# opas-lab/olearning-sim

Measured on AMD Instinct MI355X. Metric: virtual clients/sec (simulated FL rounds, FedAvg CNN), higher is better.
Workload: dtype bfloat16; 1 GPU; model=resnet18, preset=resnet-10k, clients_total=1250, clients_per_gpu=1250, local_steps=2, local_batch=16, num_classes=100, parallelism=dp1, global_batch=20000

## Files before the change

### olearning_sim_amd/models/resnet.py

```python

from __future__ import annotations

from typing import Optional

import torch

from .base import (ClientBatchedModel, Params, binit, kaiming,
                   blinear, bconv2d)

_STAGES = (64, 128, 256, 512)
_GN_GROUPS = 8


class ResNet18(ClientBatchedModel):
    name = "resnet18"
    num_classes = 100
    act_elems_per_sample = 1_600_000
    input_shape = (3, 32, 32)

    def __init__(self, num_classes: int = 100, in_ch: int = 3,
                 width_mult: float = 1.0):
        self.num_classes = num_classes
        self.in_ch = in_ch
        self.widths = [int(w * width_mult) for w in _STAGES]
# ... 27 lines not shown
                    conv(f"{pre}.down", out_c, ic, 1)
                    gn(f"{pre}.gndown", out_c)
            in_c = out_c
        p["fc.w"] = binit((w[3], self.num_classes), w[3], device, dtype, g)
        p["fc.b"] = binit((self.num_classes,), w[3], device, dtype, g)
        return p

    def _block(self, params: Params, x: torch.Tensor, C: int, pre: str,
               stride: int, has_down: bool) -> torch.Tensor:
        from ..ops.fused import groupnorm_act
        h = bconv2d(x, params[f"{pre}.c1.w"], C, stride=stride, padding=1)
        h = groupnorm_act(h, C, _GN_GROUPS, params[f"{pre}.gn1.g"],
                          params[f"{pre}.gn1.b"], relu=True)
        h = bconv2d(h, params[f"{pre}.c2.w"], C, stride=1, padding=1)
        if has_down:
            sc = bconv2d(x, params[f"{pre}.down.w"], C, stride=stride)
            sc = groupnorm_act(sc, C, _GN_GROUPS, params[f"{pre}.gndown.g"],
                               params[f"{pre}.gndown.b"])
        else:
            sc = x
        return groupnorm_act(h, C, _GN_GROUPS, params[f"{pre}.gn2.g"],
                             params[f"{pre}.gn2.b"], res=sc, relu=True)

    def _block_cbf(self, params: Params, x: torch.Tensor, C: int, pre: str,
                   stride: int, has_down: bool) -> torch.Tensor:
        from ..ops.conv import client_conv3x3, client_conv1x1
        from ..ops.fused import groupnorm_act
        h = client_conv3x3(x, params[f"{pre}.c1.w"], stride)
        h = groupnorm_act(h, C, _GN_GROUPS, params[f"{pre}.gn1.g"],
                          params[f"{pre}.gn1.b"], relu=True)
        h = client_conv3x3(h, params[f"{pre}.c2.w"], 1)
        if has_down:
            sc = client_conv1x1(x, params[f"{pre}.down.w"], stride)
            sc = groupnorm_act(sc, C, _GN_GROUPS, params[f"{pre}.gndown.g"],
                               params[f"{pre}.gndown.b"])
        else:
            sc = x
        return groupnorm_act(h, C, _GN_GROUPS, params[f"{pre}.gn2.g"],
                             params[f"{pre}.gn2.b"], res=sc, relu=True)

    def forward_cbf(self, params: Params, x: torch.Tensor) -> torch.Tensor:
        from ..ops.conv import client_conv3x3
        from ..ops.fused import groupnorm_act
        C, B = x.shape[0], x.shape[1]
        h = x.permute(0, 2, 1, 3, 4).contiguous()
        h = client_conv3x3(h, params["stem.w"], 1)
        h = groupnorm_act(h, C, _GN_GROUPS, params["stem.gn.g"],
                          params["stem.gn.b"], relu=True)
        for s in range(4):
            stride = 1 if s == 0 else 2
            h = self._block_cbf(params, h, C, f"s{s}.b0", stride, s > 0)
            h = self._block_cbf(params, h, C, f"s{s}.b1", 1, False)
        h = h.mean(dim=(3, 4)).permute(0, 2, 1)
        return blinear(h, params["fc.w"], params["fc.b"])

    def forward(self, params: Params, x: torch.Tensor) -> torch.Tensor:
        from ..ops.fused import groupnorm_act
        import os
        if x.is_cuda and x.dtype == torch.bfloat16 and \
                os.environ.get("OLSIM_CONV", "custom") == "custom":
            from ..ops.fused import hip_ops_available
            if hip_ops_available():
                return self.forward_cbf(params, x)
        C, B = x.shape[0], x.shape[1]
        h = x.permute(1, 0, 2, 3, 4).reshape(B, C * self.in_ch, 32, 32)
        h = bconv2d(h, params["stem.w"], C, stride=1, padding=1)
        h = groupnorm_act(h, C, _GN_GROUPS, params["stem.gn.g"],
                          params["stem.gn.b"], relu=True)
        for s in range(4):
            stride = 1 if s == 0 else 2
            has_down = s > 0
            h = self._block(params, h, C, f"s{s}.b0", stride, has_down)
            h = self._block(params, h, C, f"s{s}.b1", 1, False)
        h = h.mean(dim=(2, 3)).reshape(B, C, self.widths[3]).permute(1, 0, 2)
        return blinear(h, params["fc.w"], params["fc.b"])
# ... 1 lines not shown
```

### olearning_sim_amd/ops/conv.py

```python

from __future__ import annotations

import torch
import torch.nn.functional as F

from .fused import load_hip_ops


def _cpu_conv3x3(x: torch.Tensor, w: torch.Tensor, stride: int) -> torch.Tensor:
    C, IC, B, H, W = x.shape
    OC = w.shape[1]
    xg = x.permute(2, 0, 1, 3, 4).reshape(B, C * IC, H, W)
    wf = w.reshape(C * OC, IC, 3, 3)
    y = F.conv2d(xg, wf, stride=stride, padding=1, groups=C)
    OH, OW = y.shape[-2:]
    return y.reshape(B, C, OC, OH, OW).permute(1, 2, 0, 3, 4).contiguous()


class _Conv3x3Fn(torch.autograd.Function):
    @staticmethod
    def forward(ctx, x, w, stride):
        ops = load_hip_ops(required=True)
        y = ops.conv3x3_fwd(x, w, stride)
        ctx.save_for_backward(x, w)
# ... 27 lines not shown

    @staticmethod
    def forward(ctx, x, w, stride):
        ops = load_hip_ops(required=True)
        x_pad = _pad(x, 1)
        y = ops.conv3x3_fwd_p(x_pad, w, stride)
        ctx.save_for_backward(x_pad, w)
        ctx.stride = stride
        return y

    @staticmethod
    def backward(ctx, dy):
        x_pad, w = ctx.saved_tensors
        ops = load_hip_ops(required=True)
        dy = dy.contiguous()
        dx = dw = None
        H, W = x_pad.shape[3] - 2, x_pad.shape[4] - 2
        if ctx.needs_input_grad[0]:
            dy_pad = _pad(dy, 1)
            dx = ops.conv3x3_dgrad_p(dy_pad, w, H, W, ctx.stride)
        if ctx.needs_input_grad[1]:
            dw = ops.conv3x3_wgrad_p(x_pad, dy, ctx.stride)
        return dx, dw, None


def _v6_ok(ops, x: torch.Tensor, w: torch.Tensor, stride: int) -> bool:
    import os
    if os.environ.get("OLSIM_CONV_V", "") == "5":
        return False
    C, IC, B, H, W = x.shape
    return bool(ops.conv3x3_v6_ok(IC, w.shape[1], B, H, W, stride))


def client_conv3x3(x: torch.Tensor, w: torch.Tensor,
                   stride: int = 1) -> torch.Tensor:
    if x.is_cuda and x.dtype == torch.bfloat16:
        ops = load_hip_ops(required=True)
        if _v6_ok(ops, x, w, stride):
            return _Conv3x3PadFn.apply(x.contiguous(), w.contiguous(), stride)
        return _Conv3x3Fn.apply(x.contiguous(), w.contiguous(), stride)
    return _cpu_conv3x3(x, w, stride)



_NTAB_CACHE: dict = {}

# ... 94 lines not shown
    if x.is_cuda and x.dtype in (torch.bfloat16, torch.float32):
        return _Pool2x2Fn.apply(x.contiguous())
    shape = x.shape
    flat = x.reshape(-1, 1, shape[-2], shape[-1])
    out = F.max_pool2d(flat, 2)
    return out.reshape(*shape[:-2], shape[-2] // 2, shape[-1] // 2)


class _Subsample2Fn(torch.autograd.Function):

    @staticmethod
    def forward(ctx, x):
        ops = load_hip_ops(required=True)
        ctx.hw = x.shape[-2:]
        return ops.subsample2(x.contiguous())

    @staticmethod
    def backward(ctx, dy):
        ops = load_hip_ops(required=True)
        H, W = ctx.hw
        return ops.subsample2_bwd(dy.contiguous(), H, W)


def client_conv1x1(x: torch.Tensor, w: torch.Tensor,
                   stride: int = 1) -> torch.Tensor:
    C, IC, B, H, W = x.shape
    OC = w.shape[1]
    if stride != 1:
        if (stride == 2 and x.is_cuda and H % 2 == 0 and W % 4 == 0
                and x.dtype in (torch.bfloat16, torch.float32)):
            x = _Subsample2Fn.apply(x)
        else:
            x = x[:, :, :, ::stride, ::stride].contiguous()
        H, W = x.shape[-2:]
    y = torch.bmm(w.reshape(C, OC, IC), x.reshape(C, IC, B * H * W))
    return y.view(C, OC, B, H, W)
```

### olearning_sim_amd/ops/csrc/bindings.cpp

```cpp

#include <torch/extension.h>
#include <ATen/cuda/CUDAContext.h>
#include <hip/hip_runtime.h>

extern "C" void ols_fused_sgd_update_flat(
    void* buf, const void* grad, const void* master, const int64_t* offs,
    int nblocks, int64_t clients, int64_t total, float lr, float mu,
    int dtype, hipStream_t stream);

extern "C" void ols_weighted_delta_accum_flat(
    float* delta, const void* buf, const void* master, const float* weights,
    const int64_t* offs, int nblocks, int64_t clients, int64_t pglobal,
    float wsum, int dtype, hipStream_t stream);

extern "C" void ols_cross_entropy_fwd_bwd(
    const void* logits, const int64_t* labels, float* loss, void* dlogits,
    int64_t nrows, int64_t K, float inv_n, int dtype, hipStream_t stream);

extern "C" void ols_groupnorm_fwd(const void* x, const void* res, void* y,
                                  float* mean, float* rstd, const void* gamma,
                                  const void* beta, int B, int C, int ch,
                                  int G, int HW, float eps, bool relu,
                                  int layout, int dtype, hipStream_t stream);

// ... 63 lines not shown

extern "C" void ols_relu_mask(const void* dy, const void* y, void* out,
                              int64_t n, int dtype, hipStream_t stream);

extern "C" void ols_layernorm_fwd(const void* x, const void* gamma,
                                  const void* beta, void* y, float* mean,
                                  float* rstd, int64_t rows, int H,
                                  int64_t rows_per_client, float eps,
                                  int dtype, hipStream_t stream);
extern "C" void ols_layernorm_bwd(const void* x, const void* dy,
                                  const void* gamma, const float* mean,
                                  const float* rstd, void* dx, float* dgamma,
                                  float* dbeta, int64_t rows, int H,
                                  int64_t rows_per_client, int dtype,
                                  hipStream_t stream);

extern "C" void ols_groupnorm_bwd(const void* x, const void* y,
                                  const void* dy, void* dx, void* dres,
                                  const float* mean, const float* rstd,
                                  const void* gamma, float* dgamma,
                                  float* dbeta, int B, int C, int ch, int G,
                                  int HW, bool relu, int layout, int dtype,
                                  hipStream_t stream);

namespace {

int dtype_code(const at::Tensor& t) {
  switch (t.scalar_type()) {
    case at::kFloat: return 0;
    case at::kBFloat16: return 1;
    case at::kHalf: return 2;
    default:
      TORCH_CHECK(false, "olsim_hip: unsupported dtype ", t.scalar_type());
  }
}

void fused_sgd_update_flat(at::Tensor buf, at::Tensor grad,
                           at::Tensor global_flat, at::Tensor offsets,
                           int64_t clients, double lr, double mu) {
  TORCH_CHECK(buf.is_cuda() && buf.is_contiguous(), "buf must be GPU+contig");
  TORCH_CHECK(grad.sizes() == buf.sizes() && grad.scalar_type() == buf.scalar_type());
  const bool prox = mu != 0.0 && global_flat.numel() > 0;
  if (prox) {
    TORCH_CHECK(offsets.numel() >= 2 && offsets.scalar_type() == at::kLong);
    TORCH_CHECK(global_flat.scalar_type() == buf.scalar_type());
  }
// ... 348 lines not shown
  int64_t planes = x.numel() / ((int64_t)H * W);
  auto sizes = x.sizes().vec();
  sizes[sizes.size() - 2] = H / 2;
  sizes[sizes.size() - 1] = W / 2;
  auto y = at::empty(sizes, x.options());
  int dt = x.scalar_type() == at::kBFloat16 ? 1 : 0;
  ols_subsample2_fwd(x.data_ptr(), y.data_ptr(), planes, H / 2, W / 2, dt,
                     at::cuda::getCurrentCUDAStream().stream());
  return y;
}

at::Tensor subsample2_bwd(at::Tensor dy, int64_t H, int64_t W) {
  TORCH_CHECK(dy.is_cuda() && dy.is_contiguous() && dy.dim() >= 2);
  TORCH_CHECK(dy.size(-2) == H / 2 && dy.size(-1) == W / 2);
  int64_t planes = dy.numel() / ((int64_t)(H / 2) * (W / 2));
  auto sizes = dy.sizes().vec();
  sizes[sizes.size() - 2] = H;
  sizes[sizes.size() - 1] = W;
  auto dx = at::empty(sizes, dy.options());
  int dt = dy.scalar_type() == at::kBFloat16 ? 1 : 0;
  ols_subsample2_bwd(dy.data_ptr(), dx.data_ptr(), planes, (int)H, (int)W,
                     dt, at::cuda::getCurrentCUDAStream().stream());
  return dx;
}


at::Tensor replicate(at::Tensor src, int64_t clients) {
  TORCH_CHECK(src.is_cuda() && src.is_contiguous() && clients >= 1);
  TORCH_CHECK(src.numel() % 8 == 0);
  TORCH_CHECK(src.scalar_type() == at::kBFloat16 ||
              src.scalar_type() == at::kFloat);
  auto sizes = src.sizes().vec();
  sizes.insert(sizes.begin(), clients);
  auto dst = at::empty(sizes, src.options());
  int dt = src.scalar_type() == at::kBFloat16 ? 1 : 0;
  ols_replicate(src.data_ptr(), dst.data_ptr(), clients, src.numel(), dt,
                at::cuda::getCurrentCUDAStream().stream());
  return dst;
}

at::Tensor synth_batch(at::Tensor x, at::Tensor y, double s, double t) {
  TORCH_CHECK(x.is_cuda() && x.is_contiguous() && x.dim() == 2);
  TORCH_CHECK(x.scalar_type() == at::kFloat && x.size(1) % 8 == 0);
  TORCH_CHECK(y.is_cuda() && y.is_contiguous() &&
              y.scalar_type() == at::kLong);
  int64_t rows = y.numel(), batch = x.size(0), n = x.size(1);
// ... 64 lines not shown
  m.def("groupnorm_bwd(Tensor x, Tensor y, Tensor dy, Tensor mean, "
        "Tensor rstd, Tensor gamma, int clients, int groups, bool has_res, "
        "bool relu) -> (Tensor, Tensor, Tensor, Tensor)");
  m.def("mfma_selftest(Tensor A, Tensor B) -> Tensor");
  m.def("conv3x3_fwd(Tensor x, Tensor w, int stride) -> Tensor");
  m.def("conv3x3_dgrad(Tensor dy, Tensor w, int H, int W, int stride) -> Tensor");
  m.def("conv3x3_wgrad(Tensor x, Tensor dy, int stride) -> Tensor");
  m.def("conv3x3_v6_ok(int IC, int OC, int B, int H, int W, int stride) -> bool",
        &conv3x3_v6_ok);
  m.def("conv3x3_fwd_p(Tensor xp, Tensor w, int stride) -> Tensor");
  m.def("conv3x3_dgrad_p(Tensor dyp, Tensor w, int H, int W, int stride) -> Tensor");
  m.def("conv3x3_wgrad_p(Tensor xp, Tensor dy, int stride) -> Tensor");
  m.def("conv5x5_fwd(Tensor x, Tensor w, Tensor bias, Tensor ntab, bool relu) -> Tensor");
  m.def("conv5x5_dgrad(Tensor dyp, Tensor w, Tensor ntab, int H, int W) -> Tensor");
  m.def("conv5x5_wgrad(Tensor x, Tensor dy, Tensor ntab) -> Tensor");
  m.def("pool2x2_fwd(Tensor x) -> (Tensor, Tensor)");
  m.def("pool2x2_bwd(Tensor dy, Tensor arg) -> Tensor");
  m.def("transpose2d(Tensor x) -> Tensor");
  m.def("pad2d(Tensor x, int pad) -> Tensor");
  m.def("relu_mask(Tensor dy, Tensor y) -> Tensor");
  m.def("replicate(Tensor src, int clients) -> Tensor");
  m.def("subsample2(Tensor x) -> Tensor");
  m.def("subsample2_bwd(Tensor dy, int H, int W) -> Tensor");
  m.def("synth_batch(Tensor x, Tensor y, float s, float t) -> Tensor");
  m.def("layernorm_fwd(Tensor x, Tensor gamma, Tensor beta, float eps) -> (Tensor, Tensor, Tensor)");
  m.def("layernorm_bwd(Tensor x, Tensor dy, Tensor gamma, Tensor mean, Tensor rstd) -> (Tensor, Tensor, Tensor)");
}

TORCH_LIBRARY_IMPL(olsim_hip, CUDA, m) {
  m.impl("fused_sgd_update_flat", &fused_sgd_update_flat);
  m.impl("weighted_delta_accum_flat", &weighted_delta_accum_flat);
  m.impl("cross_entropy_fwd_bwd", &cross_entropy_fwd_bwd);
  m.impl("groupnorm_fwd", &groupnorm_fwd);
  m.impl("groupnorm_bwd", &groupnorm_bwd);
  m.impl("mfma_selftest", &mfma_selftest);
  m.impl("conv3x3_fwd", &conv3x3_fwd);
  m.impl("conv3x3_dgrad", &conv3x3_dgrad);
  m.impl("conv3x3_wgrad", &conv3x3_wgrad);
  m.impl("conv3x3_fwd_p", &conv3x3_fwd_p);
  m.impl("conv3x3_dgrad_p", &conv3x3_dgrad_p);
  m.impl("conv3x3_wgrad_p", &conv3x3_wgrad_p);
  m.impl("conv5x5_fwd", &conv5x5_fwd);
  m.impl("conv5x5_dgrad", &conv5x5_dgrad);
  m.impl("conv5x5_wgrad", &conv5x5_wgrad);
  m.impl("pool2x2_fwd", &pool2x2_fwd);
  m.impl("pool2x2_bwd", &pool2x2_bwd);
  m.impl("transpose2d", &transpose2d);
  m.impl("pad2d", &pad2d);
  m.impl("relu_mask", &relu_mask);
  m.impl("replicate", &replicate);
  m.impl("subsample2", &subsample2);
  m.impl("subsample2_bwd", &subsample2_bwd);
  m.impl("synth_batch", &synth_batch);
  m.impl("layernorm_fwd", &layernorm_fwd);
  m.impl("layernorm_bwd", &layernorm_bwd);
}
```

### olearning_sim_amd/ops/csrc/groupnorm.hip

```cpp

#include "common.h"

template <typename T, bool HAS_RES, bool RELU, int LAYOUT>
__global__ __launch_bounds__(OLS_THREADS) void k_gn_fwd(
    const T* __restrict__ x, const T* __restrict__ res, T* __restrict__ y,
    float* __restrict__ mean_out, float* __restrict__ rstd_out,
    const T* __restrict__ gamma, const T* __restrict__ beta,
    int Bn, int C, int ch, int G, int HW, float eps) {
  const int cg = ch / G;
  const int n = cg * HW;
  const int group = blockIdx.x;
  int c, g;
  int64_t base, pstride;
  if (LAYOUT == 0) {
    g = group % G;
    c = (group / G) % C;
    base = (int64_t)group * n;
    pstride = HW;
  } else {
    const int b = group % Bn;
    g = (group / Bn) % G;
    c = group / (Bn * G);
    base = (((int64_t)c * ch + (int64_t)g * cg) * Bn + b) * HW;
    pstride = (int64_t)Bn * HW;
// ... 404 lines not shown
  for (int v8 = threadIdx.x; v8 < nv; v8 += blockDim.x) {
    int i = v8 * 8;
    int chan = i / HW;
    int64_t idx = (LAYOUT == 0) ? i : ((int64_t)chan * pstride + i % HW);
    Pack<T, 8> px = xbuf[v8];
    Pack<T, 8> pg = gbuf[v8];
    const float ga = to_f32(gam[chan]);
    Pack<T, 8> pdx;
#pragma unroll
    for (int e = 0; e < 8; ++e) {
      float grad = to_f32(pg.v[e]);
      float xhat = (to_f32(px.v[e]) - mean) * rstd;
      float dxhat = grad * ga;
      pdx.v[e] = from_f32<T>(rstd * (dxhat - m1 - xhat * m2));
    }
    *reinterpret_cast<Pack<T, 8>*>(&dxg[idx]) = pdx;
    if (HAS_RES) *reinterpret_cast<Pack<T, 8>*>(&drg[idx]) = pg;
  }
  __syncthreads();
  for (int i = threadIdx.x; i < cg; i += blockDim.x) {
    atomicAdd(&dgamma[(int64_t)c * ch + g * cg + i], ch_dg[i]);
    atomicAdd(&dbeta[(int64_t)c * ch + g * cg + i], ch_db[i]);
  }
}

template <typename T>
static void launch_fwd(const T* x, const T* res, T* y, float* mean,
                       float* rstd, const T* gamma, const T* beta, int B,
                       int C, int ch, int G, int HW, float eps, bool relu,
                       int layout, hipStream_t s) {
  dim3 grid(B * C * G), block(OLS_THREADS);
  const bool has_res = res != nullptr;
  const int n = (ch / G) * HW;
  const size_t lds = (size_t)n * sizeof(T);
  const bool use_lds = (HW % 8) == 0 && sizeof(T) == 2 && lds <= 65536;
#define CASE(HR, RL, LY)                                                      \
  do {                                                                        \
    if (use_lds)                                                              \
      hipLaunchKernelGGL((k_gn_fwd_lds<T, HR, RL, LY>), grid, block, lds, s, \
                         x, res, y, mean, rstd, gamma, beta, B, C, ch, G,    \
                         HW, eps);                                           \
    else                                                                      \
      hipLaunchKernelGGL((k_gn_fwd<T, HR, RL, LY>), grid, block, 0, s, x,    \
                         res, y, mean, rstd, gamma, beta, B, C, ch, G, HW,   \
                         eps);                                               \
  } while (0)
// ... 82 lines not shown
```

### olearning_sim_amd/ops/csrc/pool2x2.hip

```cpp

#include "common.h"

template <typename T>
__global__ __launch_bounds__(OLS_THREADS) void k_pool2x2_fwd(
    const T* __restrict__ x, T* __restrict__ y,
    unsigned char* __restrict__ arg, int64_t n_out, int OH, int OW) {
  const int64_t stride = (int64_t)gridDim.x * blockDim.x;
  const int W = OW * 2;
  for (int64_t i = (int64_t)blockIdx.x * blockDim.x + threadIdx.x;
       i < n_out; i += stride) {
    const int64_t plane = i / (OH * OW);
    const int rem = (int)(i - plane * (OH * OW));
    const int oi = rem / OW, oj = rem - (rem / OW) * OW;
    const T* p = x + (plane * (2 * OH) + 2 * oi) * W + 2 * oj;
    float v00 = to_f32(p[0]), v01 = to_f32(p[1]);
    float v10 = to_f32(p[W]), v11 = to_f32(p[W + 1]);
    float m0 = fmaxf(v00, v01), m1 = fmaxf(v10, v11);
    float m = fmaxf(m0, m1);
    unsigned char a;
    if (m == v00) a = 0;
    else if (m == v01) a = 1;
    else if (m == v10) a = 2;
    else a = 3;
    y[i] = from_f32<T>(m);
// ... 53 lines not shown


template <typename T>
__global__ __launch_bounds__(OLS_THREADS) void k_subsample2_fwd(
    const T* __restrict__ x, T* __restrict__ y, int64_t n_out2, int OH,
    int OW) {
  const int64_t stride = (int64_t)gridDim.x * blockDim.x;
  const int W = OW * 2, OW2 = OW / 2;
  for (int64_t i = (int64_t)blockIdx.x * blockDim.x + threadIdx.x;
       i < n_out2; i += stride) {
    const int64_t plane = i / (OH * OW2);
    const int rem = (int)(i - plane * (OH * OW2));
    const int oi = rem / OW2, oj2 = (rem - (rem / OW2) * OW2) * 2;
    const T* p = x + (plane * (2 * OH) + 2 * oi) * (int64_t)W + 2 * oj2;
    Pack<T, 2> o;
    o.v[0] = p[0];
    o.v[1] = p[2];
    *reinterpret_cast<Pack<T, 2>*>(
        &y[(plane * OH + oi) * (int64_t)OW + oj2]) = o;
  }
}

template <typename T>
__global__ __launch_bounds__(OLS_THREADS) void k_subsample2_bwd(
    const T* __restrict__ dy, T* __restrict__ dx, int64_t n_in2, int H,
    int W) {
  const int64_t stride = (int64_t)gridDim.x * blockDim.x;
  const int W2 = W / 2, OW = W / 2;
  for (int64_t i = (int64_t)blockIdx.x * blockDim.x + threadIdx.x;
       i < n_in2; i += stride) {
    const int64_t plane = i / (H * W2);
    const int rem = (int)(i - plane * (H * W2));
    const int r = rem / W2, c = (rem - (rem / W2) * W2) * 2;
    Pack<T, 2> o;
    o.v[1] = from_f32<T>(0.f);
    o.v[0] = ((r & 1) == 0)
                 ? dy[(plane * (H / 2) + (r >> 1)) * (int64_t)OW + (c >> 1)]
                 : from_f32<T>(0.f);
    *reinterpret_cast<Pack<T, 2>*>(&dx[(plane * H + r) * (int64_t)W + c]) = o;
  }
}

extern "C" void ols_subsample2_fwd(const void* x, void* y, int64_t planes,
                                   int OH, int OW, int dtype,
                                   hipStream_t stream) {
  const int64_t n2 = planes * OH * (OW / 2);
  dim3 grid(ols_grid(n2, OLS_THREADS)), block(OLS_THREADS);
  if (dtype == 1)
    hipLaunchKernelGGL((k_subsample2_fwd<__hip_bfloat16>), grid, block, 0,
                       stream, (const __hip_bfloat16*)x, (__hip_bfloat16*)y,
                       n2, OH, OW);
  else
    hipLaunchKernelGGL((k_subsample2_fwd<float>), grid, block, 0, stream,
                       (const float*)x, (float*)y, n2, OH, OW);
}

extern "C" void ols_subsample2_bwd(const void* dy, void* dx, int64_t planes,
                                   int H, int W, int dtype,
                                   hipStream_t stream) {
  const int64_t n2 = planes * H * (W / 2);
  dim3 grid(ols_grid(n2, OLS_THREADS)), block(OLS_THREADS);
  if (dtype == 1)
    hipLaunchKernelGGL((k_subsample2_bwd<__hip_bfloat16>), grid, block, 0,
                       stream, (const __hip_bfloat16*)dy, (__hip_bfloat16*)dx,
                       n2, H, W);
  else
    hipLaunchKernelGGL((k_subsample2_bwd<float>), grid, block, 0, stream,
                       (const float*)dy, (float*)dx, n2, H, W);
}
```

### olearning_sim_amd/ops/fused.py

```python

from __future__ import annotations

import os
from typing import Optional, Sequence

import torch

_HIP_OPS = None
_HIP_OPS_TRIED = False

_SO_NAME = "_hip_ops.so"


def _so_path() -> str:
    return os.path.join(os.path.dirname(os.path.abspath(__file__)), _SO_NAME)


def load_hip_ops(required: bool = False):
    global _HIP_OPS, _HIP_OPS_TRIED
    if _HIP_OPS is not None:
        return _HIP_OPS
    if _HIP_OPS_TRIED and not required:
        return None
    _HIP_OPS_TRIED = True
# ... 196 lines not shown
                  gamma: torch.Tensor, beta: torch.Tensor,
                  res: Optional[torch.Tensor] = None, relu: bool = False,
                  eps: float = 1e-5) -> torch.Tensor:
    if x.is_cuda:
        return _GroupNormActFn.apply(x, res, gamma.contiguous(),
                                     beta.contiguous(), clients, groups,
                                     eps, relu)
    if x.dim() == 5:
        C, ch, B, H, W = x.shape
        cg = ch // groups
        xg = x.view(C, groups, cg, B, H, W)
        mean = xg.mean(dim=(2, 4, 5), keepdim=True)
        var = xg.var(dim=(2, 4, 5), unbiased=False, keepdim=True)
        y = ((xg - mean) * torch.rsqrt(var + eps)).view(C, ch, B, H, W)
        y = y * gamma.view(C, ch, 1, 1, 1) + beta.view(C, ch, 1, 1, 1)
    else:
        from ..models.base import bgroupnorm
        y = bgroupnorm(x, clients, groups, gamma, beta, eps)
    if res is not None:
        y = y + res
    return torch.nn.functional.relu(y) if relu else y


def fast_transpose(x: torch.Tensor) -> torch.Tensor:
    if x.is_cuda and x.dim() == 3 and \
            x.dtype in (torch.bfloat16, torch.float32):
        ops = load_hip_ops()
        if ops is not None:
            return ops.transpose2d(x.contiguous())
    return x.transpose(1, 2).contiguous()


class _LayerNormFn(torch.autograd.Function):

    @staticmethod
    def forward(ctx, x, gamma, beta, eps):
        ops = load_hip_ops(required=True)
        y, mean, rstd = ops.layernorm_fwd(x, gamma, beta, eps)
        ctx.save_for_backward(x, gamma, mean, rstd)
        return y

    @staticmethod
    def backward(ctx, dy):
        x, gamma, mean, rstd = ctx.saved_tensors
        ops = load_hip_ops(required=True)
        dx, dgamma, dbeta = ops.layernorm_bwd(x, dy.contiguous(), gamma,
# ... 16 lines not shown
```

Measured before the change: 1853 clients/s.

## Fuse GroupNorm+ReLU with padded output to feed 3x3 convs without separate pad

Adds a GroupNorm forward kernel that writes its ReLU output straight into a zero-padded buffer, plus a backward kernel that emits both the plain and the padded input gradient. These feed the padded conv3x3 forward and dgrad kernels directly. The ResNet block now threads padded activations through the network, and the stride-2 1x1 shortcut subsamples from the padded tensor. The aim is to remove the separate pad and unpad passes and their memory traffic around every conv, at the cost of a bitmask for ReLU, extra padded buffers and LDS-limited shape constraints.

New measurement: 1932 clients/s (median of 6 runs). +4.3%, better.

```diff
diff --git a/olearning_sim_amd/models/resnet.py b/olearning_sim_amd/models/resnet.py
--- a/olearning_sim_amd/models/resnet.py
+++ b/olearning_sim_amd/models/resnet.py
@@ -73,35 +73,41 @@
         return groupnorm_act(h, C, _GN_GROUPS, params[f"{pre}.gn2.g"],
                              params[f"{pre}.gn2.b"], res=sc, relu=True)
 
-    def _block_cbf(self, params: Params, x: torch.Tensor, C: int, pre: str,
-                   stride: int, has_down: bool) -> torch.Tensor:
-        from ..ops.conv import client_conv3x3, client_conv1x1
+    def _block_cbf(self, params: Params, x: torch.Tensor, x_pad, C: int,
+                   pre: str, stride: int, has_down: bool,
+                   pad_out: bool = True):
+        from ..ops.conv import conv3x3_gn_relu, client_conv1x1
         from ..ops.fused import groupnorm_act
-        h = client_conv3x3(x, params[f"{pre}.c1.w"], stride)
-        h = groupnorm_act(h, C, _GN_GROUPS, params[f"{pre}.gn1.g"],
-                          params[f"{pre}.gn1.b"], relu=True)
-        h = client_conv3x3(h, params[f"{pre}.c2.w"], 1)
+        h, h_pad = conv3x3_gn_relu(x, x_pad, params[f"{pre}.c1.w"], stride,
+                                   C, _GN_GROUPS, params[f"{pre}.gn1.g"],
+                                   params[f"{pre}.gn1.b"])
         if has_down:
-            sc = client_conv1x1(x, params[f"{pre}.down.w"], stride)
+            sc = client_conv1x1(x, params[f"{pre}.down.w"], stride,
+                                x_pad=x_pad)
             sc = groupnorm_act(sc, C, _GN_GROUPS, params[f"{pre}.gndown.g"],
                                params[f"{pre}.gndown.b"])
+            sc_pad = None
         else:
-            sc = x
-        return groupnorm_act(h, C, _GN_GROUPS, params[f"{pre}.gn2.g"],
-                             params[f"{pre}.gn2.b"], res=sc, relu=True)
+            sc, sc_pad = x, x_pad
+        return conv3x3_gn_relu(h, h_pad, params[f"{pre}.c2.w"], 1, C,
+                               _GN_GROUPS, params[f"{pre}.gn2.g"],
+                               params[f"{pre}.gn2.b"], res=sc,
+                               res_pad=sc_pad, pad_out=pad_out)
 
     def forward_cbf(self, params: Params, x: torch.Tensor) -> torch.Tensor:
         from ..ops.conv import client_conv3x3
-        from ..ops.fused import groupnorm_act
+        from ..ops.fused import groupnorm_relu_pad
         C, B = x.shape[0], x.shape[1]
         h = x.permute(0, 2, 1, 3, 4).contiguous()
         h = client_conv3x3(h, params["stem.w"], 1)
-        h = groupnorm_act(h, C, _GN_GROUPS, params["stem.gn.g"],
-                          params["stem.gn.b"], relu=True)
+        h, h_pad = groupnorm_relu_pad(h, C, _GN_GROUPS, params["stem.gn.g"],
+                                      params["stem.gn.b"])
         for s in range(4):
             stride = 1 if s == 0 else 2
-            h = self._block_cbf(params, h, C, f"s{s}.b0", stride, s > 0)
-            h = self._block_cbf(params, h, C, f"s{s}.b1", 1, False)
+            h, h_pad = self._block_cbf(params, h, h_pad, C, f"s{s}.b0",
+                                       stride, s > 0)
+            h, h_pad = self._block_cbf(params, h, h_pad, C, f"s{s}.b1", 1,
+                                       False, pad_out=s < 3)
         h = h.mean(dim=(3, 4)).permute(0, 2, 1)
         return blinear(h, params["fc.w"], params["fc.b"])
 
diff --git a/olearning_sim_amd/ops/conv.py b/olearning_sim_amd/ops/conv.py
--- a/olearning_sim_amd/ops/conv.py
+++ b/olearning_sim_amd/ops/conv.py
@@ -73,6 +73,68 @@
         if ctx.needs_input_grad[1]:
             dw = ops.conv3x3_wgrad_p(x_pad, dy, ctx.stride)
         return dx, dw, None
+
+
+class _Conv3x3GnPadFn(torch.autograd.Function):
+
+    @staticmethod
+    def forward(ctx, x, x_pad, w, res, res_pad, gamma, beta, clients,
+                groups, eps, stride, pad_out):
+        from .fused import _interior, _res_arg
+        ops = load_hip_ops(required=True)
+        h = ops.conv3x3_fwd_p(x_pad, w, stride)
+        y, mask, mean, rstd = ops.groupnorm_fwd_pad(
+            h, _res_arg(h, res, res_pad), gamma, beta, clients, groups, eps,
+            pad_out)
+        ctx.save_for_backward(x_pad, w, h, mask, mean, rstd, gamma)
+        ctx.meta = (clients, groups, res is not None, stride)
+        ctx.set_materialize_grads(False)
+        if not pad_out:
+            return y, None
+        ctx.mark_non_differentiable(y)
+        return _interior(y), y
+
+    @staticmethod
+    def backward(ctx, dy, _dy_pad):
+        x_pad, w, h, mask, mean, rstd, gamma = ctx.saved_tensors
+        clients, groups, has_res, stride = ctx.meta
+        if dy is None:
+            return (None,) * 12
+        ops = load_hip_ops(required=True)
+        need_dx = ctx.needs_input_grad[0]
+        dh, dh_pad, dres, dgamma, dbeta = ops.groupnorm_bwd_pad(
+            h, mask, dy, mean, rstd, gamma, clients, groups, has_res,
+            need_dx)
+        H, W = x_pad.shape[3] - 2, x_pad.shape[4] - 2
+        dx = dw = None
+        if need_dx:
+            dx = ops.conv3x3_dgrad_p(dh_pad, w, H, W, stride)
+        if ctx.needs_input_grad[2]:
+            dw = ops.conv3x3_wgrad_p(x_pad, dh, stride)
+        return (dx, None, dw, dres if has_res else None, None,
+                dgamma.to(gamma.dtype), dbeta.to(gamma.dtype),
+                None, None, None, None, None)
+
+
+def conv3x3_gn_relu(x: torch.Tensor, x_pad, w: torch.Tensor, stride: int,
+                    clients: int, groups: int, gamma: torch.Tensor,
+                    beta: torch.Tensor, res=None, res_pad=None,
+                    pad_out: bool = True, eps: float = 1e-5):
+    from .fused import gn_pad_shape_ok, groupnorm_act
+    if x.is_cuda and x.dtype == torch.bfloat16:
+        ops = load_hip_ops(required=True)
+        OH = (x.shape[3] + stride - 1) // stride
+        OW = (x.shape[4] + stride - 1) // stride
+        if _v6_ok(ops, x, w, stride) and gn_pad_shape_ok(w.shape[1], groups,
+                                                         OH, OW):
+            if x_pad is None:
+                x_pad = _pad(x, 1)
+            return _Conv3x3GnPadFn.apply(
+                x, x_pad, w.contiguous(), res, res_pad, gamma.contiguous(),
+                beta.contiguous(), clients, groups, eps, stride, pad_out)
+    h = client_conv3x3(x, w, stride)
+    return groupnorm_act(h, clients, groups, gamma, beta, res=res,
+                         relu=True, eps=eps), None
 
 
 def _v6_ok(ops, x: torch.Tensor, w: torch.Tensor, stride: int) -> bool:
@@ -213,14 +275,32 @@
         return ops.subsample2_bwd(dy.contiguous(), H, W)
 
 
-def client_conv1x1(x: torch.Tensor, w: torch.Tensor,
-                   stride: int = 1) -> torch.Tensor:
+class _Subsample2PadFn(torch.autograd.Function):
+
+    @staticmethod
+    def forward(ctx, x, x_pad):
+        ops = load_hip_ops(required=True)
+        ctx.hw = x.shape[-2:]
+        return ops.subsample2_p(x_pad)
+
+    @staticmethod
+    def backward(ctx, dy):
+        ops = load_hip_ops(required=True)
+        H, W = ctx.hw
+        return ops.subsample2_bwd(dy.contiguous(), H, W), None
+
+
+def client_conv1x1(x: torch.Tensor, w: torch.Tensor, stride: int = 1,
+                   x_pad=None) -> torch.Tensor:
     C, IC, B, H, W = x.shape
     OC = w.shape[1]
     if stride != 1:
         if (stride == 2 and x.is_cuda and H % 2 == 0 and W % 4 == 0
                 and x.dtype in (torch.bfloat16, torch.float32)):
-            x = _Subsample2Fn.apply(x)
+            if x_pad is not None:
+                x = _Subsample2PadFn.apply(x, x_pad)
+            else:
+                x = _Subsample2Fn.apply(x)
         else:
             x = x[:, :, :, ::stride, ::stride].contiguous()
         H, W = x.shape[-2:]
diff --git a/olearning_sim_amd/ops/csrc/bindings.cpp b/olearning_sim_amd/ops/csrc/bindings.cpp
--- a/olearning_sim_amd/ops/csrc/bindings.cpp
+++ b/olearning_sim_amd/ops/csrc/bindings.cpp
@@ -109,6 +109,21 @@
                                   float* dbeta, int B, int C, int ch, int G,
                                   int HW, bool relu, int layout, int dtype,
                                   hipStream_t stream);
+
+extern "C" int ols_gn_pad_ok(int ch, int G, int H, int W);
+extern "C" void ols_groupnorm_fwd_pad(
+    const void* x, const void* res, int res_mode, void* y, uint32_t* mask,
+    float* mean, float* rstd, const void* gamma, const void* beta, int B,
+    int C, int ch, int G, int H, int W, float eps, bool pad_out,
+    hipStream_t stream);
+extern "C" void ols_groupnorm_bwd_pad(
+    const void* x, const uint32_t* mask, const void* dy, void* dx,
+    void* dx_pad, void* dres, const float* mean, const float* rstd,
+    const void* gamma, float* dgamma, float* dbeta, int B, int C, int ch,
+    int G, int H, int W, hipStream_t stream);
+extern "C" void ols_subsample2p_fwd(const void* xp, void* y, int64_t planes,
+                                    int OH, int OW, int dtype,
+                                    hipStream_t stream);
 
 namespace {
 
@@ -503,6 +518,101 @@
   ols_subsample2_bwd(dy.data_ptr(), dx.data_ptr(), planes, (int)H, (int)W,
                      dt, at::cuda::getCurrentCUDAStream().stream());
   return dx;
+}
+
+
+bool gn_pad_ok(int64_t ch, int64_t groups, int64_t H, int64_t W) {
+  return ols_gn_pad_ok((int)ch, (int)groups, (int)H, (int)W) != 0;
+}
+
+std::tuple<at::Tensor, at::Tensor, at::Tensor, at::Tensor> groupnorm_fwd_pad(
+    at::Tensor x, at::Tensor res, at::Tensor gamma, at::Tensor beta,
+    int64_t clients, int64_t groups, double eps, bool pad_out) {
+  TORCH_CHECK(x.is_cuda() && x.is_contiguous() && x.dim() == 5);
+  TORCH_CHECK(x.scalar_type() == at::kBFloat16 &&
+              gamma.scalar_type() == at::kBFloat16 &&
+              beta.scalar_type() == at::kBFloat16);
+  TORCH_CHECK(x.size(0) == clients);
+  const int64_t ch = x.size(1), B = x.size(2), H = x.size(3), W = x.size(4);
+  TORCH_CHECK(ols_gn_pad_ok((int)ch, (int)groups, (int)H, (int)W),
+              "shape unsupported by the padded GroupNorm path");
+  TORCH_CHECK(gamma.is_contiguous() && beta.is_contiguous() &&
+              gamma.numel() == clients * ch && beta.numel() == clients * ch);
+  std::vector<int64_t> psizes = {clients, ch, B, H + 2, W + 2};
+  int res_mode = 0;
+  if (res.numel() > 0) {
+    TORCH_CHECK(res.is_cuda() && res.is_contiguous() &&
+                res.scalar_type() == at::kBFloat16);
+    if (res.sizes() == x.sizes()) res_mode = 1;
+    else if (res.sizes() == at::IntArrayRef(psizes)) res_mode = 2;
+    else TORCH_CHECK(false, "groupnorm_fwd_pad: residual shape mismatch");
+  }
+  auto y = pad_out ? at::empty(psizes, x.options()) : at::empty_like(x);
+  const int64_t ngroups = B * clients * groups;
+  const int64_t n = (ch / groups) * H * W;
+  auto mask = at::empty({ngroups, (n + 31) / 32},
+                        x.options().dtype(at::kInt));
+  auto mean = at::empty({ngroups}, x.options().dtype(at::kFloat));
+  auto rstd = at::empty({ngroups}, x.options().dtype(at::kFloat));
+  ols_groupnorm_fwd_pad(
+      x.data_ptr(), res_mode ? res.data_ptr() : nullptr, res_mode,
+      y.data_ptr(), reinterpret_cast<uint32_t*>(mask.data_ptr<int>()),
+      mean.data_ptr<float>(), rstd.data_ptr<float>(), gamma.data_ptr(),
+      beta.data_ptr(), (int)B, (int)clients, (int)ch, (int)groups, (int)H,
+      (int)W, (float)eps, pad_out,
+      at::cuda::getCurrentCUDAStream().stream());
+  return {y, mask, mean, rstd};
+}
+
+std::tuple<at::Tensor, at::Tensor, at::Tensor, at::Tensor, at::Tensor>
+groupnorm_bwd_pad(at::Tensor x, at::Tensor mask, at::Tensor dy,
+                  at::Tensor mean, at::Tensor rstd, at::Tensor gamma,
+                  int64_t clients, int64_t groups, bool has_res,
+                  bool want_pad) {
+  TORCH_CHECK(x.is_cuda() && x.is_contiguous() && x.dim() == 5);
+  TORCH_CHECK(x.scalar_type() == at::kBFloat16 &&
+              dy.scalar_type() == at::kBFloat16 && dy.sizes() == x.sizes());
+  const int64_t ch = x.size(1), B = x.size(2), H = x.size(3), W = x.size(4);
+  TORCH_CHECK(x.size(0) == clients &&
+              ols_gn_pad_ok((int)ch, (int)groups, (int)H, (int)W));
+  const int64_t ngroups = B * clients * groups;
+  const int64_t n = (ch / groups) * H * W;
+  TORCH_CHECK(mask.is_contiguous() && mask.scalar_type() == at::kInt &&
+              mask.numel() == ngroups * ((n + 31) / 32));
+  TORCH_CHECK(mean.numel() == ngroups && rstd.numel() == ngroups);
+  auto dyc = dy.contiguous();
+  auto dx = at::empty_like(x);
+  auto dx_pad = want_pad ? at::empty({clients, ch, B, H + 2, W + 2},
+                                     x.options())
+                         : at::empty({0}, x.options());
+  auto dres = has_res ? at::empty_like(x) : at::empty({0}, x.options());
+  auto dgamma = at::zeros({clients, ch}, x.options().dtype(at::kFloat));
+  auto dbeta = at::zeros({clients, ch}, x.options().dtype(at::kFloat));
+  ols_groupnorm_bwd_pad(
+      x.data_ptr(), reinterpret_cast<const uint32_t*>(mask.data_ptr<int>()),
+      dyc.data_ptr(), dx.data_ptr(), want_pad ? dx_pad.data_ptr() : nullptr,
+      has_res ? dres.data_ptr() : nullptr, mean.data_ptr<float>(),
+      rstd.data_ptr<float>(), gamma.data_ptr(), dgamma.data_ptr<float>(),
+      dbeta.data_ptr<float>(), (int)B, (int)clients, (int)ch, (int)groups,
+      (int)H, (int)W, at::cuda::getCurrentCUDAStream().stream());
+  return {dx, dx_pad, dres, dgamma, dbeta};
+}
+
+at::Tensor subsample2_p(at::Tensor xp) {
+  TORCH_CHECK(xp.is_cuda() && xp.is_contiguous() && xp.dim() >= 2);
+  int H = xp.size(-2) - 2, W = xp.size(-1) - 2;
+  TORCH_CHECK(H >= 2 && H % 2 == 0 && W % 4 == 0);
+  TORCH_CHECK(xp.scalar_type() == at::kBFloat16 ||
+              xp.scalar_type() == at::kFloat);
+  int64_t planes = xp.numel() / ((int64_t)(H + 2) * (W + 2));
+  auto sizes = xp.sizes().vec();
+  sizes[sizes.size() - 2] = H / 2;
+  sizes[sizes.size() - 1] = W / 2;
+  auto y = at::empty(sizes, xp.options());
+  int dt = xp.scalar_type() == at::kBFloat16 ? 1 : 0;
+  ols_subsample2p_fwd(xp.data_ptr(), y.data_ptr(), planes, H / 2, W / 2, dt,
+                      at::cuda::getCurrentCUDAStream().stream());
+  return y;
 }
 
 
@@ -613,6 +723,14 @@
   m.def("replicate(Tensor src, int clients) -> Tensor");
   m.def("subsample2(Tensor x) -> Tensor");
   m.def("subsample2_bwd(Tensor dy, int H, int W) -> Tensor");
+  m.def("subsample2_p(Tensor xp) -> Tensor");
+  m.def("gn_pad_ok(int ch, int groups, int H, int W) -> bool", &gn_pad_ok);
+  m.def("groupnorm_fwd_pad(Tensor x, Tensor res, Tensor gamma, Tensor beta, "
+        "int clients, int groups, float eps, bool pad_out) -> "
+        "(Tensor, Tensor, Tensor, Tensor)");
+  m.def("groupnorm_bwd_pad(Tensor x, Tensor mask, Tensor dy, Tensor mean, "
+        "Tensor rstd, Tensor gamma, int clients, int groups, bool has_res, "
+        "bool want_pad) -> (Tensor, Tensor, Tensor, Tensor, Tensor)");
   m.def("synth_batch(Tensor x, Tensor y, float s, float t) -> Tensor");
   m.def("layernorm_fwd(Tensor x, Tensor gamma, Tensor beta, float eps) -> (Tensor, Tensor, Tensor)");
   m.def("layernorm_bwd(Tensor x, Tensor dy, Tensor gamma, Tensor mean, Tensor rstd) -> (Tensor, Tensor, Tensor)");
@@ -642,6 +760,9 @@
   m.impl("replicate", &replicate);
   m.impl("subsample2", &subsample2);
   m.impl("subsample2_bwd", &subsample2_bwd);
+  m.impl("subsample2_p", &subsample2_p);
+  m.impl("groupnorm_fwd_pad", &groupnorm_fwd_pad);
+  m.impl("groupnorm_bwd_pad", &groupnorm_bwd_pad);
   m.impl("synth_batch", &synth_batch);
   m.impl("layernorm_fwd", &layernorm_fwd);
   m.impl("layernorm_bwd", &layernorm_bwd);
diff --git a/olearning_sim_amd/ops/csrc/groupnorm.hip b/olearning_sim_amd/ops/csrc/groupnorm.hip
--- a/olearning_sim_amd/ops/csrc/groupnorm.hip
+++ b/olearning_sim_amd/ops/csrc/groupnorm.hip
@@ -450,6 +450,339 @@
     atomicAdd(&dgamma[(int64_t)c * ch + g * cg + i], ch_dg[i]);
     atomicAdd(&dbeta[(int64_t)c * ch + g * cg + i], ch_db[i]);
   }
+}
+
+
+typedef __hip_bfloat16 bf16;
+
+struct __align__(8) Bf4 {
+  bf16 v[4];
+};
+
+template <int RES, bool PAD_OUT>
+__global__ __launch_bounds__(OLS_THREADS) void k_gn_fwd_pad(
+    const bf16* __restrict__ x, const bf16* __restrict__ res,
+    bf16* __restrict__ y, uint32_t* __restrict__ mask,
+    float* __restrict__ mean_out, float* __restrict__ rstd_out,
+    const bf16* __restrict__ gamma, const bf16* __restrict__ beta, int Bn,
+    int C, int ch, int G, int H, int W, float eps) {
+  const int cg = ch / G;
+  const int HW = H * W;
+  const int n = cg * HW;
+  const int PW = W + 2, PHW = (H + 2) * PW;
+  const int group = blockIdx.x;
+  const int b = group % Bn;
+  const int g = (group / Bn) % G;
+  const int c = group / (Bn * G);
+  const int64_t plane0 = ((int64_t)c * ch + (int64_t)g * cg) * Bn + b;
+  const int64_t base = plane0 * HW, pstride = (int64_t)Bn * HW;
+  const int64_t pbase = plane0 * PHW, ppstride = (int64_t)Bn * PHW;
+  const bf16* xg = x + base;
+
+  extern __shared__ __attribute__((aligned(16))) unsigned char lds_raw[];
+  Pack<bf16, 8>* xbuf = reinterpret_cast<Pack<bf16, 8>*>(lds_raw);
+  const int nv = n / 8;
+  Pack<bf16, 8>* rbuf = xbuf + nv;
+
+  __shared__ float red[2][OLS_THREADS / WAVE];
+  float s1 = 0.f, s2 = 0.f;
+  for (int v8 = threadIdx.x; v8 < nv; v8 += blockDim.x) {
+    int i = v8 * 8;
+    int64_t idx = (int64_t)(i / HW) * pstride + i % HW;
+    Pack<bf16, 8> px = *reinterpret_cast<const Pack<bf16, 8>*>(&xg[idx]);
+    xbuf[v8] = px;
+    if (RES == 1)
+      rbuf[v8] = *reinterpret_cast<const Pack<bf16, 8>*>(&res[base + idx]);
+#pragma unroll
+    for (int e = 0; e < 8; ++e) {
+      float v = to_f32(px.v[e]);
+      s1 += v;
+      s2 += v * v;
+    }
+  }
+  s1 = wave_sum(s1);
+  s2 = wave_sum(s2);
+  const int wid = threadIdx.x / WAVE, nw = blockDim.x / WAVE;
+  if ((threadIdx.x & (WAVE - 1)) == 0) { red[0][wid] = s1; red[1][wid] = s2; }
+  __syncthreads();
+  s1 = 0.f; s2 = 0.f;
+  for (int w = 0; w < nw; ++w) { s1 += red[0][w]; s2 += red[1][w]; }
+  const float mean = s1 / n;
+  const float var = fmaxf(s2 / n - mean * mean, 0.f);
+  const float rstd = rsqrtf(var + eps);
+  if (threadIdx.x == 0) { mean_out[group] = mean; rstd_out[group] = rstd; }
+
+  const bf16* gam = gamma + (int64_t)c * ch + g * cg;
+  const bf16* bet = beta + (int64_t)c * ch + g * cg;
+  bf16* xe = reinterpret_cast<bf16*>(xbuf);
+  const bf16* re = reinterpret_cast<const bf16*>(rbuf);
+  if (PAD_OUT) {
+    const int nvp = PHW / 4;
+    const int total = cg * nvp;
+    for (int t = threadIdx.x; t < total; t += blockDim.x) {
+      const int chan = t / nvp;
+      const int q = (t - chan * nvp) * 4;
+      int ph = q / PW, pw = q - ph * PW;
+      const int64_t off = pbase + (int64_t)chan * ppstride + q;
+      Bf4 pr;
+      if (RES == 2) pr = *reinterpret_cast<const Bf4*>(&res[off]);
+      const float ga = to_f32(gam[chan]), be = to_f32(bet[chan]);
+      Bf4 py;
+#pragma unroll
+      for (int e = 0; e < 4; ++e) {
+        bf16 o = from_f32<bf16>(0.f);
+        if (ph >= 1 && ph <= H && pw >= 1 && pw <= W) {
+          const int li = chan * HW + (ph - 1) * W + (pw - 1);
+          float v = (to_f32(xe[li]) - mean) * rstd;
+          v = v * ga + be;
+          if (RES == 1) v += to_f32(re[li]);
+          if (RES == 2) v += to_f32(pr.v[e]);
+          v = fmaxf(v, 0.f);
+          o = from_f32<bf16>(v);
+          xe[li] = o;
+        }
+        py.v[e] = o;
+        if (++pw == PW) { pw = 0; ++ph; }
+      }
+      *reinterpret_cast<Bf4*>(&y[off]) = py;
+    }
+  } else {
+    for (int v8 = threadIdx.x; v8 < nv; v8 += blockDim.x) {
+      int i = v8 * 8;
+      int chan = i / HW;
+      int hw = i - chan * HW;
+      int64_t idx = (int64_t)chan * pstride + hw;
+      Pack<bf16, 8> px = xbuf[v8];
+      Pack<bf16, 8> pr;
+      if (RES == 1) pr = rbuf[v8];
+      if (RES == 2) {
+        const bf16* rp = res + pbase + (int64_t)chan * ppstride;
+#pragma unroll
+        for (int e = 0; e < 8; ++e) {
+          int h = (hw + e) / W, w = (hw + e) - h * W;
+          pr.v[e] = rp[(h + 1) * PW + (w + 1)];
+        }
+      }
+      Pack<bf16, 8> py;
+      const float ga = to_f32(gam[chan]), be = to_f32(bet[chan]);
+#pragma unroll
+      for (int e = 0; e < 8; ++e) {
+        float v = (to_f32(px.v[e]) - mean) * rstd;
+        v = v * ga + be;
+        if (RES != 0) v += to_f32(pr.v[e]);
+        v = fmaxf(v, 0.f);
+        py.v[e] = from_f32<bf16>(v);
+      }
+      xbuf[v8] = py;
+      *reinterpret_cast<Pack<bf16, 8>*>(&y[base + idx]) = py;
+    }
+  }
+  __syncthreads();
+  const int nwords = (n + 31) / 32;
+  uint32_t* mg = mask + (int64_t)group * nwords;
+  for (int j = threadIdx.x; j < nwords; j += blockDim.x) {
+    uint32_t wv = 0;
+#pragma unroll
+    for (int k = 0; k < 4; ++k) {
+      const int v8 = j * 4 + k;
+      if (v8 < nv) {
+        Pack<bf16, 8> p = xbuf[v8];
+#pragma unroll
+        for (int e = 0; e < 8; ++e)
+          if (to_f32(p.v[e]) > 0.f) wv |= 1u << (k * 8 + e);
+      }
+    }
+    mg[j] = wv;
+  }
+}
+
+template <bool HAS_RES>
+__global__ __launch_bounds__(OLS_THREADS) void k_gn_bwd_pad(
+    const bf16* __restrict__ x, const uint32_t* __restrict__ mask,
+    const bf16* __restrict__ dy, bf16* __restrict__ dx,
+    bf16* __restrict__ dx_pad, bf16* __restrict__ dres,
+    const float* __restrict__ mean_in, const float* __restrict__ rstd_in,
+    const bf16* __restrict__ gamma, float* __restrict__ dgamma,
+    float* __restrict__ dbeta, int Bn, int C, int ch, int G, int H, int W) {
+  const int cg = ch / G;
+  const int HW = H * W;
+  const int n = cg * HW;
+  const int PW = W + 2, PHW = (H + 2) * PW;
+  const int group = blockIdx.x;
+  const int b = group % Bn;
+  const int g = (group / Bn) % G;
+  const int c = group / (Bn * G);
+  const int64_t plane0 = ((int64_t)c * ch + (int64_t)g * cg) * Bn + b;
+  const int64_t base = plane0 * HW, pstride = (int64_t)Bn * HW;
+  const int64_t pbase = plane0 * PHW, ppstride = (int64_t)Bn * PHW;
+  const bf16* xg = x + base;
+  const bf16* dyg_in = dy + base;
+  bf16* dxg = dx + base;
+  bf16* drg = HAS_RES ? dres + base : nullptr;
+  const float mean = mean_in[group], rstd = rstd_in[group];
+  const bf16* gam = gamma + (int64_t)c * ch + g * cg;
+  const uint32_t* mg = mask + (int64_t)group * ((n + 31) / 32);
+
+  extern __shared__ __attribute__((aligned(16))) unsigned char lds_raw[];
+  Pack<bf16, 8>* xbuf = reinterpret_cast<Pack<bf16, 8>*>(lds_raw);
+  Pack<bf16, 8>* gbuf = xbuf + n / 8;
+
+  __shared__ float red[2][OLS_THREADS / WAVE];
+  __shared__ float ch_dg[MAX_CG], ch_db[MAX_CG];
+  for (int i = threadIdx.x; i < cg; i += blockDim.x) {
+    ch_dg[i] = 0.f; ch_db[i] = 0.f;
+  }
+  __syncthreads();
+
+  const int lane = threadIdx.x & (WAVE - 1);
+  float s1 = 0.f, s2 = 0.f;
+  const int nv = n / 8;
+  const int hv = HW / 8;
+  const int lpc = min(WAVE, hv);
+  for (int v8 = threadIdx.x; v8 - lane < nv; v8 += blockDim.x) {
+    const bool active = v8 < nv;
+    int i = active ? v8 * 8 : 0;
+    int chan = i / HW;
+    int64_t idx = (int64_t)chan * pstride + i % HW;
+    float dg = 0.f, db = 0.f;
+    if (active) {
+      Pack<bf16, 8> pdy = *reinterpret_cast<const Pack<bf16, 8>*>(&dyg_in[idx]);
+      Pack<bf16, 8> px = *reinterpret_cast<const Pack<bf16, 8>*>(&xg[idx]);
+      const uint32_t mb = mg[v8 >> 2] >> ((v8 & 3) * 8);
+      const float ga = to_f32(gam[chan]);
+      Pack<bf16, 8> pg;
+#pragma unroll
+      for (int e = 0; e < 8; ++e) {
+        float grad = to_f32(pdy.v[e]);
+        grad = ((mb >> e) & 1u) ? grad : 0.f;
+        pg.v[e] = from_f32<bf16>(grad);
+        float xhat = (to_f32(px.v[e]) - mean) * rstd;
+        float dxhat = grad * ga;
+        s1 += dxhat;
+        s2 += dxhat * xhat;
+        dg += grad * xhat;
+        db += grad;
+      }
+      xbuf[v8] = px;
+      gbuf[v8] = pg;
+    }
+#pragma unroll
+    for (int off = 32; off > 0; off >>= 1)
+      if (off < lpc) {
+        dg += __shfl_xor(dg, off, WAVE);
+        db += __shfl_xor(db, off, WAVE);
+      }
+    if (active && (lane & (lpc - 1)) == 0) {
+      atomicAdd(&ch_dg[chan], dg);
+      atomicAdd(&ch_db[chan], db);
+    }
+  }
+  s1 = wave_sum(s1);
+  s2 = wave_sum(s2);
+  const int wid = threadIdx.x / WAVE, nw = blockDim.x / WAVE;
+  if ((threadIdx.x & (WAVE - 1)) == 0) { red[0][wid] = s1; red[1][wid] = s2; }
+  __syncthreads();
+  s1 = 0.f; s2 = 0.f;
+  for (int w = 0; w < nw; ++w) { s1 += red[0][w]; s2 += red[1][w]; }
+  const float m1 = s1 / n, m2 = s2 / n;
+
+  for (int v8 = threadIdx.x; v8 < nv; v8 += blockDim.x) {
+    int i = v8 * 8;
+    int chan = i / HW;
+    int64_t idx = (int64_t)chan * pstride + i % HW;
+    Pack<bf16, 8> px = xbuf[v8];
+    Pack<bf16, 8> pg = gbuf[v8];
+    const float ga = to_f32(gam[chan]);
+    Pack<bf16, 8> pdx;
+#pragma unroll
+    for (int e = 0; e < 8; ++e) {
+      float grad = to_f32(pg.v[e]);
+      float xhat = (to_f32(px.v[e]) - mean) * rstd;
+      float dxhat = grad * ga;
+      pdx.v[e] = from_f32<bf16>(rstd * (dxhat - m1 - xhat * m2));
+    }
+    *reinterpret_cast<Pack<bf16, 8>*>(&dxg[idx]) = pdx;
+    if (HAS_RES) *reinterpret_cast<Pack<bf16, 8>*>(&drg[idx]) = pg;
+    xbuf[v8] = pdx;
+  }
+  __syncthreads();
+  if (dx_pad != nullptr) {
+    const bf16* de = reinterpret_cast<const bf16*>(xbuf);
+    const int nvp = PHW / 4;
+    const int total = cg * nvp;
+    for (int t = threadIdx.x; t < total; t += blockDim.x) {
+      const int chan = t / nvp;
+      const int q = (t - chan * nvp) * 4;
+      int ph = q / PW, pw = q - ph * PW;
+      Bf4 po;
+#pragma unroll
+      for (int e = 0; e < 4; ++e) {
+        bf16 o = from_f32<bf16>(0.f);
+        if (ph >= 1 && ph <= H && pw >= 1 && pw <= W)
+          o = de[chan * HW + (ph - 1) * W + (pw - 1)];
+        po.v[e] = o;
+        if (++pw == PW) { pw = 0; ++ph; }
+      }
+      *reinterpret_cast<Bf4*>(
+          &dx_pad[pbase + (int64_t)chan * ppstride + q]) = po;
+    }
+  }
+  for (int i = threadIdx.x; i < cg; i += blockDim.x) {
+    atomicAdd(&dgamma[(int64_t)c * ch + g * cg + i], ch_dg[i]);
+    atomicAdd(&dbeta[(int64_t)c * ch + g * cg + i], ch_db[i]);
+  }
+}
+
+extern "C" int ols_gn_pad_ok(int ch, int G, int H, int W) {
+  if (G <= 0 || ch % G != 0 || ch / G > MAX_CG) return 0;
+  if (H < 2 || W < 2 || (H & 1) || (W & 1) || (H * W) % 8 != 0) return 0;
+  const int64_t n = (int64_t)(ch / G) * H * W;
+  return n * 4 <= 65536;
+}
+
+extern "C" void ols_groupnorm_fwd_pad(
+    const void* x, const void* res, int res_mode, void* y, uint32_t* mask,
+    float* mean, float* rstd, const void* gamma, const void* beta, int B,
+    int C, int ch, int G, int H, int W, float eps, bool pad_out,
+    hipStream_t s) {
+  dim3 grid(B * C * G), block(OLS_THREADS);
+  const int n = (ch / G) * H * W;
+  const size_t lds = (size_t)n * sizeof(bf16) * (res_mode == 1 ? 2 : 1);
+#define CASE(RM, PO)                                                          \
+  hipLaunchKernelGGL((k_gn_fwd_pad<RM, PO>), grid, block, lds, s,             \
+                     (const bf16*)x, (const bf16*)res, (bf16*)y, mask, mean,  \
+                     rstd, (const bf16*)gamma, (const bf16*)beta, B, C, ch,   \
+                     G, H, W, eps)
+  if (pad_out) {
+    if (res_mode == 0) CASE(0, true);
+    else if (res_mode == 1) CASE(1, true);
+    else CASE(2, true);
+  } else {
+    if (res_mode == 0) CASE(0, false);
+    else if (res_mode == 1) CASE(1, false);
+    else CASE(2, false);
+  }
+#undef CASE
+}
+
+extern "C" void ols_groupnorm_bwd_pad(
+    const void* x, const uint32_t* mask, const void* dy, void* dx,
+    void* dx_pad, void* dres, const float* mean, const float* rstd,
+    const void* gamma, float* dgamma, float* dbeta, int B, int C, int ch,
+    int G, int H, int W, hipStream_t s) {
+  dim3 grid(B * C * G), block(OLS_THREADS);
+  const int n = (ch / G) * H * W;
+  const size_t lds = (size_t)n * 2 * sizeof(bf16);
+  if (dres != nullptr)
+    hipLaunchKernelGGL((k_gn_bwd_pad<true>), grid, block, lds, s,
+                       (const bf16*)x, mask, (const bf16*)dy, (bf16*)dx,
+                       (bf16*)dx_pad, (bf16*)dres, mean, rstd,
+                       (const bf16*)gamma, dgamma, dbeta, B, C, ch, G, H, W);
+  else
+    hipLaunchKernelGGL((k_gn_bwd_pad<false>), grid, block, lds, s,
+                       (const bf16*)x, mask, (const bf16*)dy, (bf16*)dx,
+                       (bf16*)dx_pad, (bf16*)dres, mean, rstd,
+                       (const bf16*)gamma, dgamma, dbeta, B, C, ch, G, H, W);
 }
 
 template <typename T>
diff --git a/olearning_sim_amd/ops/csrc/pool2x2.hip b/olearning_sim_amd/ops/csrc/pool2x2.hip
--- a/olearning_sim_amd/ops/csrc/pool2x2.hip
+++ b/olearning_sim_amd/ops/csrc/pool2x2.hip
@@ -99,6 +99,26 @@
 }
 
 template <typename T>
+__global__ __launch_bounds__(OLS_THREADS) void k_subsample2p_fwd(
+    const T* __restrict__ xp, T* __restrict__ y, int64_t n_out2, int OH,
+    int OW) {
+  const int64_t stride = (int64_t)gridDim.x * blockDim.x;
+  const int PW = OW * 2 + 2, PH = OH * 2 + 2, OW2 = OW / 2;
+  for (int64_t i = (int64_t)blockIdx.x * blockDim.x + threadIdx.x;
+       i < n_out2; i += stride) {
+    const int64_t plane = i / (OH * OW2);
+    const int rem = (int)(i - plane * (OH * OW2));
+    const int oi = rem / OW2, oj2 = (rem - (rem / OW2) * OW2) * 2;
+    const T* p = xp + (plane * PH + 2 * oi + 1) * (int64_t)PW + 2 * oj2 + 1;
+    Pack<T, 2> o;
+    o.v[0] = p[0];
+    o.v[1] = p[2];
+    *reinterpret_cast<Pack<T, 2>*>(
+        &y[(plane * OH + oi) * (int64_t)OW + oj2]) = o;
+  }
+}
+
+template <typename T>
 __global__ __launch_bounds__(OLS_THREADS) void k_subsample2_bwd(
     const T* __restrict__ dy, T* __restrict__ dx, int64_t n_in2, int H,
     int W) {
@@ -132,6 +152,20 @@
                        (const float*)x, (float*)y, n2, OH, OW);
 }
 
+extern "C" void ols_subsample2p_fwd(const void* xp, void* y, int64_t planes,
+                                    int OH, int OW, int dtype,
+                                    hipStream_t stream) {
+  const int64_t n2 = planes * OH * (OW / 2);
+  dim3 grid(ols_grid(n2, OLS_THREADS)), block(OLS_THREADS);
+  if (dtype == 1)
+    hipLaunchKernelGGL((k_subsample2p_fwd<__hip_bfloat16>), grid, block, 0,
+                       stream, (const __hip_bfloat16*)xp, (__hip_bfloat16*)y,
+                       n2, OH, OW);
+  else
+    hipLaunchKernelGGL((k_subsample2p_fwd<float>), grid, block, 0, stream,
+                       (const float*)xp, (float*)y, n2, OH, OW);
+}
+
 extern "C" void ols_subsample2_bwd(const void* dy, void* dx, int64_t planes,
                                    int H, int W, int dtype,
                                    hipStream_t stream) {
diff --git a/olearning_sim_amd/ops/fused.py b/olearning_sim_amd/ops/fused.py
--- a/olearning_sim_amd/ops/fused.py
+++ b/olearning_sim_amd/ops/fused.py
@@ -242,6 +242,71 @@
     return torch.nn.functional.relu(y) if relu else y
 
 
+
+def gn_pad_shape_ok(ch: int, groups: int, H: int, W: int) -> bool:
+    if os.environ.get("OLSIM_GN_PAD", "1") == "0":
+        return False
+    ops = load_hip_ops(required=True)
+    return bool(ops.gn_pad_ok(ch, groups, H, W))
+
+
+def gn_pad_eligible(x: torch.Tensor, groups: int) -> bool:
+    if not (x.is_cuda and x.dtype == torch.bfloat16 and x.dim() == 5):
+        return False
+    return gn_pad_shape_ok(x.shape[1], groups, x.shape[3], x.shape[4])
+
+
+def _res_arg(x, res, res_pad):
+    if res is None:
+        return torch.empty(0, dtype=x.dtype, device=x.device)
+    return res_pad if res_pad is not None else res.contiguous()
+
+
+def _interior(y_pad: torch.Tensor) -> torch.Tensor:
+    return y_pad[..., 1:-1, 1:-1]
+
+
+class _GroupNormPadFn(torch.autograd.Function):
+
+    @staticmethod
+    def forward(ctx, x, res, res_pad, gamma, beta, clients, groups, eps):
+        ops = load_hip_ops(required=True)
+        y_pad, mask, mean, rstd = ops.groupnorm_fwd_pad(
+            x, _res_arg(x, res, res_pad), gamma, beta, clients, groups, eps,
+            True)
+        ctx.save_for_backward(x, mask, mean, rstd, gamma)
+        ctx.meta = (clients, groups, res is not None)
+        ctx.mark_non_differentiable(y_pad)
+        ctx.set_materialize_grads(False)
+        return _interior(y_pad), y_pad
+
+    @staticmethod
+    def backward(ctx, dy, _dy_pad):
+        x, mask, mean, rstd, gamma = ctx.saved_tensors
+        clients, groups, has_res = ctx.meta
+        if dy is None:
+            return (None,) * 8
+        ops = load_hip_ops(required=True)
+        dx, _, dres, dgamma, dbeta = ops.groupnorm_bwd_pad(
+            x, mask, dy, mean, rstd, gamma, clients, groups, has_res, False)
+        return (dx, dres if has_res else None, None,
+                dgamma.to(gamma.dtype), dbeta.to(gamma.dtype),
+                None, None, None)
+
+
+def groupnorm_relu_pad(x: torch.Tensor, clients: int, groups: int,
+                       gamma: torch.Tensor, beta: torch.Tensor,
+                       res: Optional[torch.Tensor] = None,
+                       res_pad: Optional[torch.Tensor] = None,
+                       eps: float = 1e-5):
+    if gn_pad_eligible(x, groups):
+        return _GroupNormPadFn.apply(x.contiguous(), res, res_pad,
+                                     gamma.contiguous(), beta.contiguous(),
+                                     clients, groups, eps)
+    return groupnorm_act(x, clients, groups, gamma, beta, res=res,
+                         relu=True, eps=eps), None
+
+
 def fast_transpose(x: torch.Tensor) -> torch.Tensor:
     if x.is_cuda and x.dim() == 3 and \
             x.dtype in (torch.bfloat16, torch.float32):
```
